# dropbox/divans

Hardware: AMD Instinct MI355X
Metric: MB/s encode+decode per GPU, 64 KiB metablocks; bit-exact vs CPU (higher is better)
Workload: dtype u16/u64 integer

## Files before the change

### divans_amd/csrc/capi.cpp

```cpp
#include <hip/hip_runtime.h>

#include <algorithm>
#include <atomic>
#include <cstdio>
#include <cstdlib>
#include <cstring>
#include <mutex>
#include <string>
#include <vector>

#include "../../include/divans_gpu.h"
#include "lit_kernels.h"
#include "lit_device.h"

using namespace divans_hip;

static thread_local std::string g_last_error;
static int fail(int code, const std::string& msg) { g_last_error = msg; return code; }
#define HIP_TRY(expr)                                                                              \
    do {                                                                                           \
        hipError_t e_ = (expr);                                                                    \
        if (e_ != hipSuccess)                                                                      \
            return fail(DIVANS_GPU_EHIP, std::string(#expr) + ": " + hipGetErrorString(e_));       \
    } while (0)
// ... 64 lines not shown
static void make_luts(uint8_t mode, uint8_t* lut0, uint8_t* lut1) {
    for (int i = 0; i < 256; ++i) {
        switch (mode) {
        case 3: lut0[i] = (uint8_t)(signed3(i) << 3); lut1[i] = signed3(i); break;
        case 2: lut0[i] = utf8_lut0(i); lut1[i] = utf8_lut1(i); break;
        case 1: lut0[i] = (uint8_t)(i >> 2); lut1[i] = 0; break;
        default: lut0[i] = (uint8_t)(i & 0x3f); lut1[i] = 0; break;
        }
    }
}

struct TableMem { int16_t* p = nullptr; size_t bytes = 0; std::vector<hipMemGenericAllocationHandle_t> chunks; size_t chunk_bytes = 0, va_bytes = 0; int device = 0; };

struct divans_gpu_codec {
    int device = 0;
    hipStream_t stream = nullptr;
    divans_lit_config cfg;
    LitGeometry geom;
    bool mix = false;
    uint32_t max_stream_len = 0;
    uint32_t num_cus = 256;
    uint32_t blocks = 0;
    uint32_t cache_high = 0, cache_low = 0;
    bool cache_unified = false;
    uint32_t decode_gen = 2;
#ifndef DIVANS_DM_AUTO_DEFAULT
#define DIVANS_DM_AUTO_DEFAULT 1
#endif
    bool dm_auto = DIVANS_DM_AUTO_DEFAULT != 0;
    uint32_t dm_log2 = 0, dm_shift = 0;
    uint32_t blocks2 = 0;
    uint32_t blocks_t = 0, t_log2 = 0, t_shift = 0;
    bool user_geometry = false;
    char last_decode_kernel[128] = "";
    uint32_t last_decode_grid = 0;
    uint8_t* d_stream_flags = nullptr;
    uint8_t* d_blob = nullptr;
    int16_t* d_tables = nullptr;  size_t tables_bytes = 0;
    TableMem tm;
    uint32_t byte_order = 0;
    uint8_t* d_rank = nullptr;
    bool rank_ready = false;
    uint32_t rans_split = 0;
    uint32_t table_candidates = 0; bool tables_tuned = false;
    bool eager_tune = false;
    divans_gpu_table_placement placement = {0u, 0u, 0.f, 0.f, 0.f, 0u, 0u};
    struct PlacementSearch {
        bool active = false, pending = false;
        uint32_t sig_streams = 0, sig_len = 0;
        TableMem best_tm;
        float best_ms = 0.f, worst_ms = 0.f;
        hipEvent_t e0 = nullptr, e1 = nullptr;
        uint64_t seq_at_measure = 0;
    } ps;
    uint64_t table_launch_seq = 0;
    uint32_t* d_sf = nullptr;     size_t sf_bytes = 0;
    uint32_t* d_status = nullptr;
    bool bucket_ok = false;
    bool bucket_mix_ok = false;
    uint32_t bucket_mix_batch = 32768;
    uint8_t* d_slots = nullptr; size_t slots_bytes = 0;
    uint64_t* d_slot_off = nullptr; size_t slot_off_cap = 0;
    std::vector<hipEvent_t> ev_span; size_t enc_spans = 0;
    float last_pack_ms = 0;
    uint32_t encode_path = 0;
    uint32_t last_encode_path = 0;
// ... 681 lines not shown
extern "C" int divans_gpu_codec_table_placement(divans_gpu_codec* c, divans_gpu_table_placement* out) {
    if (!c || !out) return fail(DIVANS_GPU_EINVAL, "null argument");
    *out = c->placement;
    out->policy_candidates = table_candidates_of(c);
    out->searching = (c->ps.active && !c->tables_tuned) ? 1u : 0u;
    return 0;
}

extern "C" int divans_gpu_table_memory(divans_gpu_table_memory_info* out) {
    if (!out) return fail(DIVANS_GPU_EINVAL, "null argument");
    out->va_reserved_bytes = g_va_reserved.load(); out->va_cap_bytes = g_va_cap.load();
    std::lock_guard<std::mutex> lock(g_table_pool_mu);
    out->idle_ranges = (uint32_t)g_table_pool.size(); out->idle_bytes = 0;
    for (const TableMem& m : g_table_pool) out->idle_bytes += m.va_bytes;
    return 0;
}
extern "C" void divans_gpu_set_table_va_cap(uint64_t bytes) { g_va_cap.store(bytes); }

static bool valid_cache_rows(uint32_t r) { return r == 0 || (r >= 16 && r <= 256 && (r & (r - 1)) == 0); }

extern "C" int divans_gpu_codec_set_geometry(divans_gpu_codec* c, uint32_t blocks, uint32_t cache_rows) {
    if (!c) return fail(DIVANS_GPU_EINVAL, "null codec");
    c->user_geometry = true;
    if (cache_rows != 0xffffffffu) {
        if (!valid_cache_rows(cache_rows)) return fail(DIVANS_GPU_EINVAL, "cache_rows must be 0 or a power of two in [16, 256]");
        if (cache_rows && c->geom.total_rows >= 0x7fffu) return fail(DIVANS_GPU_EINVAL, "row cache needs fewer than 32767 rows per stream");
        c->cache_high = cache_rows; c->cache_low = 0; c->cache_unified = cache_rows != 0;
#if DIVANS_WITH_EXPERIMENTAL_DECODERS
        c->decode_gen = 1;
#endif
    }
    if (blocks) {
        c->blocks = blocks;
        if (c->blocks2) {
            const uint32_t gen = c->decode_gen;
            int rc = set_decoder_impl(c, (c->dm_shift >> 31) ? 3 : 2, nullptr, nullptr, blocks, false); if (rc) return rc;
            c->decode_gen = gen;
        }
    }
    return 0;
}

extern "C" int divans_gpu_codec_set_split_cache(divans_gpu_codec* c, uint32_t high_rows, uint32_t low_rows) {
    if (!c) return fail(DIVANS_GPU_EINVAL, "null codec");
    if (!valid_cache_rows(high_rows) || !valid_cache_rows(low_rows)) return fail(DIVANS_GPU_EINVAL, "cache rows must be 0 or a power of two in [16, 256]");
    if (high_rows == 0 && low_rows != 0) return fail(DIVANS_GPU_EINVAL, "a low-nibble cache needs a high-nibble cache");
    if ((high_rows || low_rows) && c->geom.total_rows >= 0x7fffu) return fail(DIVANS_GPU_EINVAL, "row cache needs fewer than 32767 rows per stream");
    c->cache_high = high_rows; c->cache_low = low_rows; c->cache_unified = false;
#if DIVANS_WITH_EXPERIMENTAL_DECODERS
    c->decode_gen = 1;
#endif
    c->user_geometry = true;
    return 0;
}

extern "C" size_t divans_gpu_lit_encode_bound(size_t n) {
    const size_t nsym = 2 * n;
    const size_t nchunks = (nsym + 65535) / 65536;
    const size_t words = (15 * nsym + 31) / 32 + 2 * nchunks;
    const size_t bytes = 16 * nchunks + 4 * words;
    return (bytes + 15) & ~(size_t)15;
}

template <class Batch>
static void fill_bucket_batch(const divans_gpu_codec* c, uint32_t stream_len, const divans_lit_segment* d_segs, Batch& k) {
    k.stream_len = stream_len; k.max_stream_len = c->max_stream_len;
    k.pieces = bucket_pieces(c); k.slot = bucket_slot(c);
    k.segs = (const LitSegment*)d_segs; k.bt_first = c->geom.bt_first; k.n_btypes = c->geom.n_btypes; k.status = c->d_status;
}

template <class Batch, class Launch, class After>
static int bucket_sub_batches(divans_gpu_codec* c, Batch& k, uint32_t sub, const SfView& view, const uint8_t* d_in, const uint64_t* d_in_offsets,
                              const uint32_t* d_in_sizes, const uint32_t* d_seg_begin, uint32_t n_streams, Launch&& launch, After&& after) {
    HIP_TRY(hipEventRecord(c->ev[0], c->stream));
    for (uint32_t s0 = 0; s0 < n_streams; s0 += sub) {
        k.n_streams = std::min(sub, n_streams - s0);
        k.in = d_in_offsets ? d_in : d_in + (size_t)s0 * k.stream_len;
        k.in_offsets = d_in_offsets ? d_in_offsets + s0 : nullptr;
        k.in_sizes = d_in_sizes ? d_in_sizes + s0 : nullptr;
        k.seg_begin = d_seg_begin ? d_seg_begin + s0 : nullptr;
        if (int rc = launch(k)) return rc;
        if (int rc = after(s0, k.n_streams, view)) return rc;
    }
    return 0;
}

template <class After>
static int model_pass(divans_gpu_codec* c, const uint8_t* d_in, const uint64_t* d_in_offsets, const uint32_t* d_in_sizes,
                      uint32_t stream_len, uint32_t n_streams, const uint32_t* d_seg_begin, const divans_lit_segment* d_segs, After&& after) {
    int rc = maybe_learn_rank(c, d_in, d_in_offsets, d_in_sizes, n_streams, stream_len);
    if (rc) return rc;
    SfView view;
    const bool segs_ok = !d_segs || c->encode_path == 2u;
    if (use_bucket(c) && n_streams < (1u << 24) && segs_ok) {
        BucketBatch k;
        std::memset(&k, 0, sizeof(k));
        const uint32_t sub = std::min(n_streams, c->bucket_mix_batch);
        rc = ensure_bucket(c, sub, k); if (rc) return rc;
        fill_bucket_batch(c, stream_len, d_segs, k);
        k.sf = (uint32_t*)k.sfs; k.sf_stride = 2u * k.slot;
        k.inc = c->geom.inc0; k.lim = c->geom.lim0;
        c->last_encode_path = 2u;
        view.sf = k.sf; view.stride = k.sf_stride;
        view.spare = (uint8_t*)k.inv; view.spare_bytes = (size_t)sub * k.slot * 3u;
        return bucket_sub_batches(c, k, sub, view, d_in, d_in_offsets, d_in_sizes, d_seg_begin, n_streams,
                                  [&](const BucketBatch& kk) -> int { HIP_TRY(launch_bucket_model(kk, c->num_cus * 4u, c->stream)); return 0; }, after);
    }
    if (use_bucket_mix(c) && segs_ok) {
        MixBucketBatch k;
        std::memset(&k, 0, sizeof(k));
        uint32_t sub = std::min(n_streams, c->bucket_mix_batch);
        while ((rc = ensure_bucket_mix(c, sub, k)) == DIVANS_GPU_ENOMEM && sub > 1024u) { (void)hipGetLastError(); sub = (sub + 1u) / 2u; }
        if (rc) return rc;
        fill_bucket_batch(c, stream_len, d_segs, k);
        k.blob = c->d_blob; k.pos_stride = k.slot;
        k.sf = (uint32_t*)k.xs[0]; k.sf_stride = 2u * k.slot;
        k.inc0 = c->geom.inc0; k.lim0 = c->geom.lim0; k.inc2 = c->geom.inc2; k.lim2 = c->geom.lim2; k.inc3 = c->geom.inc3; k.lim3 = c->geom.lim3;
        c->last_encode_path = 3u;
        view.sf = k.sf; view.stride = k.sf_stride;
        view.spare = (uint8_t*)k.inv; view.spare_bytes = (size_t)sub * k.slot * 4u;
        return bucket_sub_batches(c, k, sub, view, d_in, d_in_offsets, d_in_sizes, d_seg_begin, n_streams,
                                  [&](const MixBucketBatch& kk) -> int { HIP_TRY(launch_bucket_mix_model(kk, c->num_cus, c->stream)); return 0; }, after);
    }
    rc = ensure_sf(c, n_streams); if (rc) return rc;
    rc = ensure_tables(c); if (rc) return rc;
    LitBatch b;
    std::memset(&b, 0, sizeof(b));
    b.blob = c->d_blob; b.geom = c->geom; b.tables = c->d_tables;
    b.n_streams = n_streams; b.stream_len = stream_len; b.max_stream_len = c->max_stream_len;
    b.in = d_in; b.in_offsets = d_in_offsets; b.in_sizes = d_in_sizes;
    b.sf = c->d_sf; b.status = c->d_status;
    b.seg_begin = d_seg_begin; b.segs = (const LitSegment*)d_segs;
    set_cache_fields(c, b);
    if (d_segs && b.cache_mode != 2u && b.cache_mode != 0u) return fail(DIVANS_GPU_EINVAL, "segment lists need the default (high-nibble-row) cache or none");
    HIP_TRY(hipEventRecord(c->ev[0], c->stream));
    ++c->table_launch_seq;
    c->last_encode_path = 1u;
    HIP_TRY(launch_model_encode(b, c->mix, c->blocks, c->stream));
    view.sf = c->d_sf; view.stride = 2u * c->max_stream_len;
    return after(0u, n_streams, view);
}

static int rans_event_pair(divans_gpu_codec* c, size_t i, hipEvent_t*& pair) {
    while (c->ev_rans.size() < 2u * (i + 1u)) {
        hipEvent_t e = nullptr;
        HIP_TRY(hipEventCreate(&e));
        c->ev_rans.push_back(e);
    }
    pair = &c->ev_rans[2u * i];
    return 0;
}

static int rans_pass(divans_gpu_codec* c, const SfView& v, uint32_t count, uint32_t stream_len, const uint32_t* d_in_sizes, uint8_t* out, uint64_t out_base,
                     uint64_t out_slot, uint64_t* d_out_offsets, uint32_t* d_out_sizes, uint32_t* d_chunk_bytes, uint32_t max_chunks, size_t& pairs) {
    const bool chunk_lanes = c->max_stream_len > 32768u && c->max_stream_len <= 65536u;
// ... 909 lines not shown
```

### divans_amd/csrc/lit_bucket.hip

```cpp
#include "lit_bucket_dev.h"

#ifndef DIVANS_BK_CHAIN_NO_STORES
#define DIVANS_BK_CHAIN_NO_STORES 0
#endif

namespace divans_hip {

template <bool SEG>
__global__ __launch_bounds__(BK_SORT_THREADS) void bucket_sort_kernel(const BucketBatch b) {
    __shared__ __attribute__((aligned(16))) unsigned long long staging64[BK_PIECE / 8u];
    uint8_t* staging = (uint8_t*)staging64;
    __shared__ __attribute__((aligned(16))) uint8_t piece_in[16 + BK_PIECE];
    __shared__ uint32_t hist[4][256];
    __shared__ uint32_t wsum[4];
    __shared__ uint8_t prev_of[SEG ? BK_PIECE : 1u];
    const uint32_t s = blockIdx.x / b.pieces, piece = blockIdx.x % b.pieces;
    const uint32_t tid = threadIdx.x, w = (uint32_t)__builtin_amdgcn_readfirstlane((int)(tid >> 6)), lane = tid & 63;
    const uint32_t len = b.in_sizes ? b.in_sizes[s] : b.stream_len;
    const uint8_t* in = b.in + (b.in_offsets ? b.in_offsets[s] : (uint64_t)s * b.stream_len);
    uint32_t* desc = b.desc + ((size_t)s * 256u + tid) * 8u + piece;
    const uint32_t base = piece * BK_PIECE;
    if (base >= len) {
        *desc = 0u;
        if (SEG && piece == 0u)
// ... 90 lines not shown
        uint32_t wbase = 0;
        if ((int)(threadIdx.x & 63u) == leader) wbase = atomicAdd(&cnt[c], (uint32_t)__popcll(m));
        wbase = (uint32_t)__builtin_amdgcn_readlane((int)wbase, leader);
        if (cls == c) local = wbase + lanes_below(m);
    }
    __syncthreads();
    if (threadIdx.x < BK_CLASSES) basev[threadIdx.x] = cnt[threadIdx.x] ? atomicAdd(&b.counters[threadIdx.x], cnt[threadIdx.x]) : 0u;
    __syncthreads();
    if (cls >= 0) b.tasks[(size_t)cls * cap + basev[cls] + local] = t;
}

constexpr uint32_t BK_LANE_DWORDS = 148;
constexpr uint32_t BK_DESC_DW = 136;
constexpr uint32_t BK_TAB_DW = 64 * BK_LANE_DWORDS;
__global__ __launch_bounds__(64) void bucket_chain_kernel(const BucketBatch b) {
    extern __shared__ __attribute__((aligned(16))) uint32_t lds32[];
    const uint32_t lane = threadIdx.x;
    uint32_t* my = lds32 + lane * BK_LANE_DWORDS;
    uint32_t* mydesc = my + BK_DESC_DW;
    uint32_t* tab = lds32 + BK_TAB_DW;
    const uint32_t inc = (uint32_t)b.inc; const int lim = b.lim;
    for (uint32_t i = lane; i < 128u; i += 64u) {
        tab[i] = bk_tab_entry(i, inc);
    }
    __syncthreads();
    const size_t pl = b.slot;
    const uint32_t cap = b.n_streams * 256u;
    BkTaskLists lists; lists.load(b.counters);
    const uint32_t total = lists.total();

    bool has_task = false, exhausted = false;
    uint32_t run_i = 0, nruns = 0, left = 0, idx = 0;
    u32x2* cur_sfs = b.sfs; const uint8_t* cur_sorted = b.sorted;
    uint32_t nt_stage = 0, nt_tid = 0;
    u32x4 nd0 = {0u, 0u, 0u, 0u}, nd1 = {0u, 0u, 0u, 0u};
    uint32_t win_cur = 0, win_end = 0, nxt_val = 0, nxt_w = 0;
    const uint32_t long_end = lists.ends[3];
    bool nxt_pending = false, drained = false;
    u32x2 e_next = {0u, 0u}; uint32_t m_next = 0;
    u32x2 pv0 = {0u, 0u}, pv1 = pv0, pv2 = pv0, pv3 = pv0, pv4 = pv0, pv5 = pv0, pv6 = pv0, pv7 = pv0;
    uint32_t m_prev = 0; u32x2* sfs_prev = b.sfs;

#define BK_OPAQUE(X) asm volatile("" : "+v"(X))
#define BK_BYTE(K, WORD, PV)                                                                            \
    if (((K - first) & 15u) < cnt) {                                                                    \
        const uint32_t byte_ = (WORD >> (8u * (K & 3u))) & 0xffu;                                       \
        const uint32_t hi = byte_ >> 4, lo = byte_ & 15u;                                               \
        uint32_t* rowl = my + 8u * (1u + hi);                                                           \
        BkRow H = bk_read(my, tab, hi), L = bk_read(rowl, tab, lo);                                     \
        const u32x2 v = {bk_pack(H, hi), bk_pack(L, lo)};                                               \
        bk_add(H); bk_add(L);                                                                           \
        bk_renorm_at(H, lim); bk_renorm_at(L, lim);                                                     \
        *(u32x4*)my = H.w0; *(u32x4*)(my + 4) = H.w1; *(u32x4*)rowl = L.w0; *(u32x4*)(rowl + 4) = L.w1; \
        PV = v;                                                                                         \
    }

    for (;;) {
        u32x2 e = e_next; const uint32_t m = m_next;
#if DIVANS_BK_CHAIN_NO_STORES
        asm volatile("" : : "v"(pv0), "v"(pv1), "v"(pv2), "v"(pv3), "v"(pv4), "v"(pv5), "v"(pv6), "v"(pv7), "v"(sfs_prev));
        if (false) {
#else
        if (m_prev & BK_VALID) {
#endif
            bk_store_group(sfs_prev, m_prev, pv0, pv1, pv2, pv3, pv4, pv5, pv6, pv7);
        }
        {
            const bool adv = has_task && left == 0u, more = run_i < nruns;
            const uint32_t d = mydesc[run_i & 7u];
            if (adv && more) { left = d >> 16; idx = d & 0xffffu; ++run_i; }
            if (adv && !more) has_task = false;
        }
        {
            const bool fetch_ = has_task && left != 0u;
            const uint32_t base = idx & ~7u, first_ = idx & 7u;
            const uint32_t cnt_ = left < 8u - first_ ? left : 8u - first_;
            const uint8_t* lp = fetch_ ? cur_sorted + base : b.sorted;
            e_next = *(const u32x2*)lp;
            m_next = fetch_ ? (base | (first_ << 16) | (cnt_ << 20) | BK_VALID) : 0u;
            idx += fetch_ ? cnt_ : 0u; left -= fetch_ ? cnt_ : 0u;
        }
        BK_OPAQUE(e);
        m_prev = m; sfs_prev = cur_sfs;
        if (m & BK_VALID) {
            const uint32_t first = (m >> 16) & 15u, cnt = (m >> 20) & 15u;
            BK_BYTE(0u, e.x, pv0) BK_BYTE(1u, e.x, pv1) BK_BYTE(2u, e.x, pv2) BK_BYTE(3u, e.x, pv3)
            BK_BYTE(4u, e.y, pv4) BK_BYTE(5u, e.y, pv5) BK_BYTE(6u, e.y, pv6) BK_BYTE(7u, e.y, pv7)
        }
        if (!has_task && !(m_next & BK_VALID) && nt_stage == 3u) {
            BK_OPAQUE(nd0); BK_OPAQUE(nd1);
            uint32_t n = 0;
            const uint32_t dsc[8] = {nd0.x, nd0.y, nd0.z, nd0.w, nd1.x, nd1.y, nd1.z, nd1.w};
#pragma unroll
            for (uint32_t j = 0; j < 8u; ++j) if (dsc[j] >> 16) { mydesc[n] = dsc[j] + j * BK_PIECE; ++n; }
            nruns = n; run_i = 0u;
            bk_rows_reset(my, 17u);
            cur_sfs = b.sfs + (size_t)(nt_tid >> 8) * pl; cur_sorted = b.sorted + (size_t)(nt_tid >> 8) * pl;
            left = 0u; has_task = true; nt_stage = 0u;
        }
        const bool want = nt_stage == 0u && !exhausted;
        if (nt_stage == 2u) nt_stage = 3u;
        else if (nt_stage == 1u) {
            BK_OPAQUE(nt_tid);
            const u32x4* dp = (const u32x4*)(b.desc + (size_t)nt_tid * 8u);
            nd0 = dp[0]; nd1 = dp[1];
            nt_stage = 2u;
        }
        const unsigned long long wm = __ballot(want);
        if (wm) {
            if (win_cur == win_end && nxt_pending) {
                BK_OPAQUE(nxt_val);
                const uint32_t basev = (uint32_t)__builtin_amdgcn_readfirstlane((int)nxt_val);
                nxt_pending = false;
                if (basev >= total) { drained = true; win_cur = win_end = total; }
                else { win_cur = basev; win_end = basev + nxt_w < total ? basev + nxt_w : total; }
            }
            const uint32_t avail = win_end - win_cur, asked = (uint32_t)__popcll(wm);
            const uint32_t rank = lanes_below(wm);
            if (want) {
                if (rank < avail) {
                    const uint32_t t = win_cur + rank;
                    nt_tid = *lists.at(b.tasks, cap, t);
                    nt_stage = 1u;
                } else if (drained) exhausted = true;
            }
            win_cur += asked < avail ? asked : avail;
        }
        const uint32_t want_w = win_end < long_end ? 64u : BK_WINDOW;
        if (!nxt_pending && !drained && win_end - win_cur < want_w / 2u) {
            nxt_w = want_w;
            if (lane == 0u) nxt_val = atomicAdd(&b.counters[BK_CLAIM], want_w);
            nxt_pending = true;
        }
        const bool done = !has_task && !(m_next & BK_VALID) && !(m_prev & BK_VALID) && nt_stage == 0u && exhausted;
        if (__ballot(!done) == 0ull) break;
    }
#undef BK_BYTE
#undef BK_OPAQUE
}

__global__ __launch_bounds__(1024) void bucket_unsort_kernel(const BucketBatch b) {
    __shared__ u32x2 buf[BK_PIECE];
    const uint32_t s = blockIdx.x / b.pieces, piece = blockIdx.x % b.pieces;
    const uint32_t len = b.in_sizes ? b.in_sizes[s] : b.stream_len;
    const uint32_t base = piece * BK_PIECE;
    if (base >= len) return;
    const uint32_t n = len - base < BK_PIECE ? len - base : BK_PIECE;
    const size_t pl = b.slot;
    const u32x2* src = b.sfs + (size_t)s * pl + base;
    for (uint32_t i = threadIdx.x; i < n; i += 1024u) buf[i] = __builtin_nontemporal_load(src + i);
    __syncthreads();
    const uint16_t* inv = b.inv + (size_t)s * pl + base;
    u32x2* dst = (u32x2*)(b.sf + (size_t)s * b.sf_stride) + base;
    for (uint32_t i = threadIdx.x; i < n; i += 1024u) dst[i] = buf[inv[i]];
}

__global__ __launch_bounds__(1024) void bucket_unsort32_kernel(const BucketBatch b) {
    __shared__ uint32_t buf[BK_PIECE];
    const uint32_t s = blockIdx.x / b.pieces, piece = blockIdx.x % b.pieces;
    const uint32_t len = b.in_sizes ? b.in_sizes[s] : b.stream_len;
    const uint32_t base = piece * BK_PIECE;
    if (base >= len) return;
    const uint32_t n = len - base < BK_PIECE ? len - base : BK_PIECE;
    const size_t pl = b.slot;
    const uint32_t* src = (const uint32_t*)b.sfs + (size_t)s * pl + base;
    const uint32_t n2 = (n + 1u) & ~1u;
    for (uint32_t i = 2u * threadIdx.x; i < n2; i += 2048u) *(u32x2*)(buf + i) = __builtin_nontemporal_load((const u32x2*)(src + i));
// ... 44 lines not shown
```

### divans_amd/csrc/lit_bucket_dev.h

```cpp
#ifndef DIVANS_LIT_BUCKET_DEV_H_
#define DIVANS_LIT_BUCKET_DEV_H_
#include "lit_device.h"

namespace divans_hip {

constexpr uint32_t BK_PIECE = 8192;
constexpr uint32_t BK_SORT_THREADS = 256;
constexpr uint32_t BK_VALID = 1u << 31;
constexpr uint32_t BK_WINDOW = 256;
constexpr uint32_t BK_CLASSES = 6;
constexpr uint32_t BK_CLAIM = 8;

__device__ __forceinline__ int bk_class_of(uint32_t tot) {
    return tot == 0u ? -1 : (tot >= 16384u ? 0 : (tot >= 8192u ? 1 : (tot >= 4096u ? 2 : (tot >= 2048u ? 3 : (tot >= 64u ? 4 : 5)))));
}
struct BkTaskLists {
    uint32_t ends[BK_CLASSES];
    __device__ __forceinline__ void load(const uint32_t* counters) {
        uint32_t acc = 0;
#pragma unroll
        for (uint32_t c = 0; c < BK_CLASSES; ++c) { acc += counters[c]; ends[c] = acc; }
    }
    __device__ __forceinline__ uint32_t total() const { return ends[BK_CLASSES - 1u]; }
    __device__ __forceinline__ const uint32_t* at(const uint32_t* tasks, uint32_t cap, uint32_t t) const {
// ... 119 lines not shown
template <class T>
__device__ __forceinline__ void bk_store_group(T* plane, uint32_t m, T r0, T r1, T r2, T r3, T r4, T r5, T r6, T r7) {
    T* dst = plane + (m & 0xffffu);
    const uint32_t pf = (m >> 16) & 15u, pc = (m >> 20) & 15u;
    if (pc == 8u) {
        bk_store_full(dst, r0, r1, r2, r3, r4, r5, r6, r7);
    } else {
        if (((0u - pf) & 15u) < pc) bk_store_one(dst + 0, r0);
        if (((1u - pf) & 15u) < pc) bk_store_one(dst + 1, r1);
        if (((2u - pf) & 15u) < pc) bk_store_one(dst + 2, r2);
        if (((3u - pf) & 15u) < pc) bk_store_one(dst + 3, r3);
        if (((4u - pf) & 15u) < pc) bk_store_one(dst + 4, r4);
        if (((5u - pf) & 15u) < pc) bk_store_one(dst + 5, r5);
        if (((6u - pf) & 15u) < pc) bk_store_one(dst + 6, r6);
        if (((7u - pf) & 15u) < pc) bk_store_one(dst + 7, r7);
    }
}

#define BK_OPAQUE(X) asm volatile("" : "+v"(X))

template <class K, class Batch>
__device__ __forceinline__ void bk_chain_loop(const typename K::Env env, const Batch b) {
    const uint32_t lane = threadIdx.x;
    uint32_t* my = env.my;
    uint32_t* mydesc = my + 8u * K::ROWS;
    const size_t pl = b.slot;
    const uint32_t cap = b.n_streams * 256u;
    BkTaskLists lists; lists.load(b.counters);
    const uint32_t total = lists.total();

    bool has_task = false, exhausted = false;
    uint32_t run_i = 0, nruns = 0, left = 0, idx = 0;
    typename K::Slot cur = K::slot(b, 0u); const auto* cur_sorted = b.sorted;
    uint32_t nt_stage = 0, nt_tid = 0;
    u32x4 nd0 = {0u, 0u, 0u, 0u}, nd1 = {0u, 0u, 0u, 0u};
    uint32_t win_cur = 0, win_end = 0, nxt_val = 0, nxt_w = 0;
    const uint32_t long_end = lists.ends[3];
    bool nxt_pending = false, drained = false;
    typename K::Group e_next = {}; uint32_t m_next = 0;
    typename K::Out out = {};
    uint32_t m_prev = 0; typename K::Slot prev = cur;

    for (;;) {
        typename K::Group e = e_next; const uint32_t m = m_next;
        if (m_prev & BK_VALID) K::store(prev, m_prev, out);
        {
            const bool adv = has_task && left == 0u, more = run_i < nruns;
            const uint32_t d = mydesc[run_i & 7u];
            if (adv && more) { left = d >> 16; idx = d & 0xffffu; ++run_i; }
            if (adv && !more) has_task = false;
        }
        {
            const bool fetch_ = has_task && left != 0u;
            const uint32_t base = idx & ~7u, first_ = idx & 7u;
            const uint32_t cnt_ = left < 8u - first_ ? left : 8u - first_;
            const auto* lp = fetch_ ? cur_sorted + base : b.sorted;
            e_next = *(const typename K::Group*)lp;
            m_next = fetch_ ? (base | (first_ << 16) | (cnt_ << 20) | BK_VALID) : 0u;
            idx += fetch_ ? cnt_ : 0u; left -= fetch_ ? cnt_ : 0u;
        }
        BK_OPAQUE(e);
        m_prev = m; prev = cur;
        if (m & BK_VALID) out = K::code(env, e, (m >> 16) & 15u, (m >> 20) & 15u, out);
        if (!has_task && !(m_next & BK_VALID) && nt_stage == 3u) {
            BK_OPAQUE(nd0); BK_OPAQUE(nd1);
            uint32_t n = 0;
            const uint32_t dsc[8] = {nd0.x, nd0.y, nd0.z, nd0.w, nd1.x, nd1.y, nd1.z, nd1.w};
#pragma unroll
            for (uint32_t j = 0; j < 8u; ++j) if (dsc[j] >> 16) { mydesc[n] = dsc[j] + j * BK_PIECE; ++n; }
            nruns = n; run_i = 0u;
            bk_rows_reset(my, K::ROWS);
            const size_t off = (size_t)(nt_tid >> 8) * pl;
            cur = K::slot(b, off); cur_sorted = b.sorted + off;
            left = 0u; has_task = true; nt_stage = 0u;
        }
        const bool want = nt_stage == 0u && !exhausted;
        if (nt_stage == 2u) nt_stage = 3u;
        else if (nt_stage == 1u) {
            BK_OPAQUE(nt_tid);
            const u32x4* dp = (const u32x4*)(b.desc + (size_t)nt_tid * 8u);
            nd0 = dp[0]; nd1 = dp[1];
            nt_stage = 2u;
        }
        const unsigned long long wm = __ballot(want);
        if (wm) {
            if (win_cur == win_end && nxt_pending) {
                BK_OPAQUE(nxt_val);
                const uint32_t basev = (uint32_t)__builtin_amdgcn_readfirstlane((int)nxt_val);
                nxt_pending = false;
                if (basev >= total) { drained = true; win_cur = win_end = total; }
                else { win_cur = basev; win_end = basev + nxt_w < total ? basev + nxt_w : total; }
            }
            const uint32_t avail = win_end - win_cur, asked = (uint32_t)__popcll(wm);
            const uint32_t rank = lanes_below(wm);
            if (want) {
                if (rank < avail) {
                    const uint32_t t = win_cur + rank;
                    nt_tid = *lists.at(b.tasks, cap, t);
                    nt_stage = 1u;
                } else if (drained) exhausted = true;
            }
            win_cur += asked < avail ? asked : avail;
        }
        const uint32_t want_w = win_end < long_end ? 64u : BK_WINDOW;
        if (!nxt_pending && !drained && win_end - win_cur < want_w / 2u) {
            nxt_w = want_w;
            if (lane == 0u) nxt_val = atomicAdd(&b.counters[BK_CLAIM], want_w);
            nxt_pending = true;
        }
        const bool done = !has_task && !(m_next & BK_VALID) && !(m_prev & BK_VALID) && nt_stage == 0u && exhausted;
        if (__ballot(!done) == 0ull) break;
    }
}
#undef BK_OPAQUE

}
#endif
```

### divans_amd/csrc/lit_bucket_mix.hip

```cpp
#include "lit_bucket_dev.h"

namespace divans_hip {

constexpr uint32_t MX_CHAIN_WAVES = 3;

template <int MODEL> struct MxGeom {
    static constexpr uint32_t NH = MODEL == 0 ? 8u : 1u;
    static constexpr uint32_t NR = NH + 16u;
    static constexpr uint32_t LANE_DW = MODEL == 0 ? 204u : 148u;
    static constexpr uint32_t LDS_BYTES = (64u * LANE_DW + 256u) * 4u;
};

template <int MODEL, bool SEG>
__global__ __launch_bounds__(BK_SORT_THREADS) void mix_sort_kernel(const MixBucketBatch b) {
    __shared__ __attribute__((aligned(16))) uint16_t staging[BK_PIECE];
    __shared__ __attribute__((aligned(16))) uint8_t piece_in[16 + BK_PIECE];
    __shared__ uint16_t kp[BK_PIECE];
    __shared__ uint32_t hist[4][256];
    __shared__ uint32_t scan[256];
    __shared__ uint8_t lut1c[256], ctxf[2048], slot_of[2048];
    const uint32_t s = blockIdx.x / b.pieces, piece = blockIdx.x % b.pieces;
    const uint32_t tid = threadIdx.x, w = tid >> 6, lane = tid & 63;
    const uint32_t len = b.in_sizes ? b.in_sizes[s] : b.stream_len;
    const uint8_t* in = b.in + (b.in_offsets ? b.in_offsets[s] : (uint64_t)s * b.stream_len);
// ... 302 lines not shown
                const uint32_t sf = bk_pack(R, s);
                rec[0] = (int)(sf & 0xffffu); rec[1] = (int)(sf >> 16); rec[2] = (int)s;
            } else if (kind == 6u) {
                bk_rows_reset(rows[0], 2u);
                for (int i = 0; i < 16; ++i) rec[i] = r0[i];
            } else if (kind == 8u && op.y < 2u) {
                ((uint16_t*)rows[op.y])[op.z & 15u] = (uint16_t)op.w;
                for (int i = 0; i < 16; ++i) rec[i] = ((const uint16_t*)rows[op.y])[i];
            } else if (kind == 10u) {
                const BkRow C = bk_read(rows[0], tab, sym), S = bk_read(rows[1], tab, sym);
                const uint32_t cm_x = (uint32_t)C.chi | (sym ? (uint32_t)C.cprev << 16 : 0u), st_x = (uint32_t)S.chi | (sym ? (uint32_t)S.cprev << 16 : 0u);
                uint32_t mf = 0u;
                const uint32_t sf = mix_nibble<true>(w, st_x, S.w1.w >> 16, cm_x, C.w1.w >> 16, &mf);
                rec[0] = (int)(sf & 0xffffu); rec[1] = (int)(sf >> 16); rec[2] = (int)sym; rec[3] = (int)(mf & 0xffffu); rec[4] = (int)(mf >> 16);
                rec[5] = w.w0; rec[6] = w.w1; rec[7] = w.norm;
            }
            if (kind == 5u || (kind == 8u && op.y >= 2u)) { rec[0] = w.w0; rec[1] = w.w1; rec[2] = w.norm; }
#pragma unroll
            for (int i = 0; i < 16; ++i) out[(size_t)k * 16u + (uint32_t)i] = rec[i];
        }
        if (kind == 10u) {
            w.w0 = __builtin_amdgcn_readfirstlane(w.w0); w.w1 = __builtin_amdgcn_readfirstlane(w.w1); w.norm = __builtin_amdgcn_readfirstlane(w.norm);
        }
    }
}

hipError_t launch_selftest_cdf_ops_bucket(const uint32_t* d_ops, uint32_t n, int32_t* d_out, hipStream_t st) {
    hipLaunchKernelGGL(cdf_ops_selftest_bucket_kernel, dim3(1), dim3(64), 0, st, (const u32x4*)d_ops, n, d_out);
    return hipGetLastError();
}

static void launch_mix_sort_seg(int model, const MixBucketBatch& b, hipStream_t st);

hipError_t launch_bucket_mix_model(const MixBucketBatch& b, uint32_t num_cus, hipStream_t st) {
    BucketBatch v;
    v.in = b.in; v.in_offsets = b.in_offsets; v.in_sizes = b.in_sizes;
    v.n_streams = b.n_streams; v.stream_len = b.stream_len; v.max_stream_len = b.max_stream_len; v.pieces = b.pieces;
    v.slot = b.slot; v.sf_stride = 2u * b.pos_stride;
    v.sorted = nullptr; v.inv = b.inv; v.desc = b.desc; v.sfs = nullptr; v.sf = nullptr; v.tasks = b.tasks; v.counters = b.counters;
    v.inc = 0; v.lim = 0;
    v.seg_begin = nullptr; v.segs = nullptr; v.bt_first = 0; v.n_btypes = 0; v.status = nullptr;
    for (int model = 0; model < 2; ++model) {
        hipError_t e = hipMemsetAsync(b.counters, 0, 64, st);
        if (e != hipSuccess) return e;
        if (b.pieces < 8u) {
            e = hipMemsetAsync(b.desc, 0, (size_t)b.n_streams * 256u * 8u * sizeof(uint32_t), st);
            if (e != hipSuccess) return e;
        }
        if (model == 0) {
            if (b.segs) launch_mix_sort_seg(0, b, st);
            else hipLaunchKernelGGL((mix_sort_kernel<0, false>), dim3(b.n_streams * b.pieces), dim3(BK_SORT_THREADS), 0, st, b);
            launch_bucket_tasks(v, st);
            hipLaunchKernelGGL(mix_chain_kernel<0>, dim3(num_cus * MX_CHAIN_WAVES), dim3(64), MxGeom<0>::LDS_BYTES, st, b);
        } else {
            if (b.segs) launch_mix_sort_seg(1, b, st);
            else hipLaunchKernelGGL((mix_sort_kernel<1, false>), dim3(b.n_streams * b.pieces), dim3(BK_SORT_THREADS), 0, st, b);
            launch_bucket_tasks(v, st);
            hipLaunchKernelGGL(mix_chain_kernel<1>, dim3(num_cus * MX_CHAIN_WAVES), dim3(64), MxGeom<1>::LDS_BYTES, st, b);
        }
        v.sfs = b.xs[model]; v.sf = (uint32_t*)b.xs[model]; v.sf_stride = 2u * b.pos_stride;
        launch_bucket_unsort(v, st);
        v.sfs = (bk_u32x2*)b.maxes[model]; v.sf = b.maxes[model]; v.sf_stride = b.pos_stride;
        launch_bucket_unsort32(v, st);
    }
    if ((b.n_streams + 31u) / 32u > num_cus * 4u) hipLaunchKernelGGL(mix_weights_kernel<2>, dim3((b.n_streams + 31u) / 32u), dim3(64), 0, st, b);
    else hipLaunchKernelGGL(mix_weights_kernel<1>, dim3((b.n_streams + 31u) / 32u), dim3(64), 0, st, b);
    return hipGetLastError();
}

static void launch_mix_sort_seg(int model, const MixBucketBatch& b, hipStream_t st) {
    if (model == 0) hipLaunchKernelGGL((mix_sort_kernel<0, true>), dim3(b.n_streams * b.pieces), dim3(BK_SORT_THREADS), 0, st, b);
    else hipLaunchKernelGGL((mix_sort_kernel<1, true>), dim3(b.n_streams * b.pieces), dim3(BK_SORT_THREADS), 0, st, b);
}

}
```

### divans_amd/csrc/lit_kernels.h

```cpp
#ifndef DIVANS_LIT_KERNELS_H_
#define DIVANS_LIT_KERNELS_H_
#include <hip/hip_runtime.h>
#include <stdint.h>

namespace divans_hip {

constexpr int LIT_THREADS = 256;
constexpr int RANS_THREADS = 64;

constexpr uint32_t LIT_BLOB_LUT1CLASS = 0;
constexpr uint32_t LIT_BLOB_CTXF = 256;
constexpr uint32_t LIT_CTXF_BYTES = 2048;
constexpr uint32_t LIT_MAX_BTYPES = 8;
constexpr uint32_t LIT_BLOB_MAX_BYTES = 256 + LIT_CTXF_BYTES * LIT_MAX_BTYPES + 8192;

struct LitGeometry {
    uint32_t nctx;
    uint32_t low_width;
    uint32_t plane0, plane1, plane2;
    uint32_t low_base;
    uint32_t cm_base;
    uint32_t total_rows;
    int32_t mm_uniform;
    int32_t ctx_const;
// ... 60 lines not shown
    int32_t inc, lim;
    const uint32_t* seg_begin;
    const LitSegment* segs;
    uint32_t bt_first, n_btypes;
    uint32_t* status;
};
hipError_t launch_bucket_model(const BucketBatch& b, uint32_t chain_blocks, hipStream_t st);
void launch_bucket_tasks(const BucketBatch& b, hipStream_t st);
void launch_bucket_unsort(const BucketBatch& b, hipStream_t st);
void launch_bucket_unsort32(const BucketBatch& b, hipStream_t st);

struct MixBucketBatch {
    const uint8_t* in; const uint64_t* in_offsets; const uint32_t* in_sizes;
    uint32_t n_streams, stream_len, max_stream_len;
    uint32_t pieces;
    uint32_t slot;
    uint32_t pos_stride;
    uint32_t sf_stride;
    const uint8_t* blob;
    uint16_t* sorted;
    uint16_t* inv;
    uint32_t* desc;
    uint32_t* tasks;
    uint32_t* counters;
    bk_u32x2* xs[2];
    uint32_t* maxes[2];
    uint32_t* sf;
    int32_t inc0, lim0, inc2, lim2, inc3, lim3;
    const uint32_t* seg_begin;
    const LitSegment* segs;
    uint32_t bt_first, n_btypes;
    uint32_t* status;
};
hipError_t launch_bucket_mix_model(const MixBucketBatch& b, uint32_t num_cus, hipStream_t st);

uint32_t lit_lds_bytes(const LitBatch& b);
hipError_t launch_model_encode(const LitBatch& b, bool mix, uint32_t blocks, hipStream_t st);
hipError_t launch_rans_encode(const RansBatch& b, hipStream_t st);
hipError_t launch_decode(const LitBatch& b, bool mix, uint32_t blocks, hipStream_t st);
hipError_t launch_decode2(const LitBatch& b, bool mix, uint32_t blocks, hipStream_t st);
void lit_decode_kernel_name(const LitBatch& b, bool mix, char* buf, size_t cap);
void lit_decode2_kernel_name(const LitBatch& b, bool mix, char* buf, size_t cap);
uint32_t lit_decode2_effective_caches(uint32_t dm_log2, bool mix, bool seg);
uint32_t lit_decode2_stream_lds(uint32_t dm_log2);
#ifndef DIVANS_WITH_EXPERIMENTAL_DECODERS
#define DIVANS_WITH_EXPERIMENTAL_DECODERS 0
#endif
#if DIVANS_WITH_EXPERIMENTAL_DECODERS
hipError_t launch_decode_t(const LitBatch& b, bool mix, uint32_t blocks, hipStream_t st);
hipError_t launch_selftest_cdf_ops_t(const uint32_t* d_ops, uint32_t n, int32_t* d_out, hipStream_t st);
void lit_decode_t_kernel_name(const LitBatch& b, bool mix, char* buf, size_t cap);
uint32_t lit_decode_t_stream_lds(uint32_t dm_log2, bool mix);
#endif
hipError_t launch_pack(const uint8_t* slots, const uint64_t* src_off, const uint32_t* sizes, uint32_t n, uint8_t* packed,
                       uint64_t* dst_off, uint64_t* total, hipStream_t st, bool accumulate = false, uint64_t cap = ~0ull, uint32_t* status = nullptr);
hipError_t launch_learn_byte_rank(const uint8_t* data, const uint64_t* offsets, const uint32_t* sizes, uint32_t n_streams, uint32_t stream_len,
                                  uint32_t sample_streams, uint32_t sample_len, uint8_t* rank, hipStream_t st);
hipError_t launch_row_replay(const LitBatch& b, bool mix, uint32_t blocks, hipStream_t st);
hipError_t launch_selftest_division(unsigned long long* d_mismatches, hipStream_t st);
hipError_t launch_selftest_cdf_ops(const uint32_t* d_ops, uint32_t n, int32_t* d_out, hipStream_t st);
hipError_t launch_selftest_cdf_ops2(const uint32_t* d_ops, uint32_t n, int32_t* d_out, hipStream_t st);
hipError_t launch_selftest_cdf_ops_bucket(const uint32_t* d_ops, uint32_t n, int32_t* d_out, hipStream_t st);

}
#endif
```

Measured before the change: 14880.

## Add one-deep task descriptor queue to bucket chain kernels; cap chain grid

Restructures the per-wave task fetch state machine in the bucket and mix-bucket chain loops. A descriptor that has finished loading is now moved into a one-entry queue, so the next task claim and its descriptor load can start while the current task is still running, instead of waiting in a stage-3 hold. The aim is to hide task-fetch latency between tasks, at the cost of more registers per lane. Separately, a user-set block count now also caps the chain kernel grid size.

```diff
diff --git a/divans_amd/csrc/capi.cpp b/divans_amd/csrc/capi.cpp
--- a/divans_amd/csrc/capi.cpp
+++ b/divans_amd/csrc/capi.cpp
@@ -120,6 +120,7 @@
     uint32_t blocks2 = 0;
     uint32_t blocks_t = 0, t_log2 = 0, t_shift = 0;
     bool user_geometry = false;
+    uint32_t chain_grid_cap = 0;
     char last_decode_kernel[128] = "";
     uint32_t last_decode_grid = 0;
     uint8_t* d_stream_flags = nullptr;
@@ -867,6 +868,7 @@
     }
     if (blocks) {
         c->blocks = blocks;
+        c->chain_grid_cap = blocks;
         if (c->blocks2) {
             const uint32_t gen = c->decode_gen;
             int rc = set_decoder_impl(c, (c->dm_shift >> 31) ? 3 : 2, nullptr, nullptr, blocks, false); if (rc) return rc;
@@ -896,6 +898,8 @@
     const size_t bytes = 16 * nchunks + 4 * words;
     return (bytes + 15) & ~(size_t)15;
 }
+
+static uint32_t chain_grid(const divans_gpu_codec* c, uint32_t own) { return c->chain_grid_cap ? std::min(own, c->chain_grid_cap) : own; }
 
 template <class Batch>
 static void fill_bucket_batch(const divans_gpu_codec* c, uint32_t stream_len, const divans_lit_segment* d_segs, Batch& k) {
@@ -939,7 +943,7 @@
         view.sf = k.sf; view.stride = k.sf_stride;
         view.spare = (uint8_t*)k.inv; view.spare_bytes = (size_t)sub * k.slot * 3u;
         return bucket_sub_batches(c, k, sub, view, d_in, d_in_offsets, d_in_sizes, d_seg_begin, n_streams,
-                                  [&](const BucketBatch& kk) -> int { HIP_TRY(launch_bucket_model(kk, c->num_cus * 4u, c->stream)); return 0; }, after);
+                                  [&](const BucketBatch& kk) -> int { HIP_TRY(launch_bucket_model(kk, chain_grid(c, c->num_cus * 4u), c->stream)); return 0; }, after);
     }
     if (use_bucket_mix(c) && segs_ok) {
         MixBucketBatch k;
@@ -955,7 +959,7 @@
         view.sf = k.sf; view.stride = k.sf_stride;
         view.spare = (uint8_t*)k.inv; view.spare_bytes = (size_t)sub * k.slot * 4u;
         return bucket_sub_batches(c, k, sub, view, d_in, d_in_offsets, d_in_sizes, d_seg_begin, n_streams,
-                                  [&](const MixBucketBatch& kk) -> int { HIP_TRY(launch_bucket_mix_model(kk, c->num_cus, c->stream)); return 0; }, after);
+                                  [&](const MixBucketBatch& kk) -> int { HIP_TRY(launch_bucket_mix_model(kk, c->num_cus, c->chain_grid_cap, c->stream)); return 0; }, after);
     }
     rc = ensure_sf(c, n_streams); if (rc) return rc;
     rc = ensure_tables(c); if (rc) return rc;
diff --git a/divans_amd/csrc/lit_bucket.hip b/divans_amd/csrc/lit_bucket.hip
--- a/divans_amd/csrc/lit_bucket.hip
+++ b/divans_amd/csrc/lit_bucket.hip
@@ -146,8 +146,9 @@
     bool has_task = false, exhausted = false;
     uint32_t run_i = 0, nruns = 0, left = 0, idx = 0;
     u32x2* cur_sfs = b.sfs; const uint8_t* cur_sorted = b.sorted;
-    uint32_t nt_stage = 0, nt_tid = 0;
-    u32x4 nd0 = {0u, 0u, 0u, 0u}, nd1 = {0u, 0u, 0u, 0u};
+    uint32_t nt_stage = 0, nt_tid = 0, q_tid = 0;
+    u32x4 nd0 = {0u, 0u, 0u, 0u}, nd1 = nd0, qd0 = nd0, qd1 = nd0;
+    bool q_full = false;
     uint32_t win_cur = 0, win_end = 0, nxt_val = 0, nxt_w = 0;
     const uint32_t long_end = lists.ends[3];
     bool nxt_pending = false, drained = false;
@@ -179,6 +180,47 @@
 #endif
             bk_store_group(sfs_prev, m_prev, pv0, pv1, pv2, pv3, pv4, pv5, pv6, pv7);
         }
+        if (nt_stage == 2u && !q_full) {
+            qd0 = nd0; qd1 = nd1; q_tid = nt_tid;
+            q_full = true; nt_stage = 0u;
+        }
+        {
+            const bool want = nt_stage == 0u && !exhausted && !q_full;
+            if (nt_stage == 1u) {
+                BK_OPAQUE(nt_tid);
+                const u32x4* dp = (const u32x4*)(b.desc + (size_t)nt_tid * 8u);
+                nd0 = dp[0]; nd1 = dp[1];
+                nt_stage = 2u;
+            }
+            const unsigned long long wm = __ballot(want);
+            if (wm) {
+                if (win_cur == win_end && nxt_pending) {
+                    BK_OPAQUE(nxt_val);
+                    const uint32_t basev = (uint32_t)__builtin_amdgcn_readfirstlane((int)nxt_val);
+                    nxt_pending = false;
+                    if (basev >= total) { drained = true; win_cur = win_end = total; }
+                    else { win_cur = basev; win_end = basev + nxt_w < total ? basev + nxt_w : total; }
+                }
+                const uint32_t avail = win_end - win_cur, asked = (uint32_t)__popcll(wm);
+                const uint32_t rank = lanes_below(wm);
+                if (want) {
+                    if (rank < avail) {
+                        const uint32_t t = win_cur + rank;
+                        nt_tid = *lists.at(b.tasks, cap, t);
+                        nt_stage = 1u;
+                    } else if (drained) exhausted = true;
+                }
+                win_cur += asked < avail ? asked : avail;
+            }
+            const uint32_t want_w = win_end < long_end ? 64u : BK_WINDOW;
+            if (!nxt_pending && !drained && win_end - win_cur < want_w / 2u) {
+                nxt_w = want_w;
+                uint32_t claim = BK_CLAIM;
+                BK_OPAQUE(claim);
+                if (lane == 0u) nxt_val = atomicAdd(b.counters + claim, want_w);
+                nxt_pending = true;
+            }
+        }
         {
             const bool adv = has_task && left == 0u, more = run_i < nruns;
             const uint32_t d = mydesc[run_i & 7u];
@@ -201,52 +243,18 @@
             BK_BYTE(0u, e.x, pv0) BK_BYTE(1u, e.x, pv1) BK_BYTE(2u, e.x, pv2) BK_BYTE(3u, e.x, pv3)
             BK_BYTE(4u, e.y, pv4) BK_BYTE(5u, e.y, pv5) BK_BYTE(6u, e.y, pv6) BK_BYTE(7u, e.y, pv7)
         }
-        if (!has_task && !(m_next & BK_VALID) && nt_stage == 3u) {
-            BK_OPAQUE(nd0); BK_OPAQUE(nd1);
+        if (!has_task && !(m_next & BK_VALID) && q_full) {
+            BK_OPAQUE(qd0); BK_OPAQUE(qd1);
             uint32_t n = 0;
-            const uint32_t dsc[8] = {nd0.x, nd0.y, nd0.z, nd0.w, nd1.x, nd1.y, nd1.z, nd1.w};
+            const uint32_t dsc[8] = {qd0.x, qd0.y, qd0.z, qd0.w, qd1.x, qd1.y, qd1.z, qd1.w};
 #pragma unroll
             for (uint32_t j = 0; j < 8u; ++j) if (dsc[j] >> 16) { mydesc[n] = dsc[j] + j * BK_PIECE; ++n; }
             nruns = n; run_i = 0u;
             bk_rows_reset(my, 17u);
-            cur_sfs = b.sfs + (size_t)(nt_tid >> 8) * pl; cur_sorted = b.sorted + (size_t)(nt_tid >> 8) * pl;
-            left = 0u; has_task = true; nt_stage = 0u;
-        }
-        const bool want = nt_stage == 0u && !exhausted;
-        if (nt_stage == 2u) nt_stage = 3u;
-        else if (nt_stage == 1u) {
-            BK_OPAQUE(nt_tid);
-            const u32x4* dp = (const u32x4*)(b.desc + (size_t)nt_tid * 8u);
-            nd0 = dp[0]; nd1 = dp[1];
-            nt_stage = 2u;
-        }
-        const unsigned long long wm = __ballot(want);
-        if (wm) {
-            if (win_cur == win_end && nxt_pending) {
-                BK_OPAQUE(nxt_val);
-                const uint32_t basev = (uint32_t)__builtin_amdgcn_readfirstlane((int)nxt_val);
-                nxt_pending = false;
-                if (basev >= total) { drained = true; win_cur = win_end = total; }
-                else { win_cur = basev; win_end = basev + nxt_w < total ? basev + nxt_w : total; }
-            }
-            const uint32_t avail = win_end - win_cur, asked = (uint32_t)__popcll(wm);
-            const uint32_t rank = lanes_below(wm);
-            if (want) {
-                if (rank < avail) {
-                    const uint32_t t = win_cur + rank;
-                    nt_tid = *lists.at(b.tasks, cap, t);
-                    nt_stage = 1u;
-                } else if (drained) exhausted = true;
-            }
-            win_cur += asked < avail ? asked : avail;
-        }
-        const uint32_t want_w = win_end < long_end ? 64u : BK_WINDOW;
-        if (!nxt_pending && !drained && win_end - win_cur < want_w / 2u) {
-            nxt_w = want_w;
-            if (lane == 0u) nxt_val = atomicAdd(&b.counters[BK_CLAIM], want_w);
-            nxt_pending = true;
-        }
-        const bool done = !has_task && !(m_next & BK_VALID) && !(m_prev & BK_VALID) && nt_stage == 0u && exhausted;
+            cur_sfs = b.sfs + (size_t)(q_tid >> 8) * pl; cur_sorted = b.sorted + (size_t)(q_tid >> 8) * pl;
+            left = 0u; has_task = true; q_full = false;
+        }
+        const bool done = !has_task && !(m_next & BK_VALID) && !(m_prev & BK_VALID) && nt_stage == 0u && !q_full && exhausted;
         if (__ballot(!done) == 0ull) break;
     }
 #undef BK_BYTE
diff --git a/divans_amd/csrc/lit_bucket_dev.h b/divans_amd/csrc/lit_bucket_dev.h
--- a/divans_amd/csrc/lit_bucket_dev.h
+++ b/divans_amd/csrc/lit_bucket_dev.h
@@ -175,8 +175,9 @@
     bool has_task = false, exhausted = false;
     uint32_t run_i = 0, nruns = 0, left = 0, idx = 0;
     typename K::Slot cur = K::slot(b, 0u); const auto* cur_sorted = b.sorted;
-    uint32_t nt_stage = 0, nt_tid = 0;
-    u32x4 nd0 = {0u, 0u, 0u, 0u}, nd1 = {0u, 0u, 0u, 0u};
+    uint32_t nt_stage = 0, nt_tid = 0, q_tid = 0;
+    u32x4 nd0 = {0u, 0u, 0u, 0u}, nd1 = nd0, qd0 = nd0, qd1 = nd0;
+    bool q_full = false;
     uint32_t win_cur = 0, win_end = 0, nxt_val = 0, nxt_w = 0;
     const uint32_t long_end = lists.ends[3];
     bool nxt_pending = false, drained = false;
@@ -187,6 +188,47 @@
     for (;;) {
         typename K::Group e = e_next; const uint32_t m = m_next;
         if (m_prev & BK_VALID) K::store(prev, m_prev, out);
+        if (nt_stage == 2u && !q_full) {
+            qd0 = nd0; qd1 = nd1; q_tid = nt_tid;
+            q_full = true; nt_stage = 0u;
+        }
+        {
+            const bool want = nt_stage == 0u && !exhausted && !q_full;
+            if (nt_stage == 1u) {
+                BK_OPAQUE(nt_tid);
+                const u32x4* dp = (const u32x4*)(b.desc + (size_t)nt_tid * 8u);
+                nd0 = dp[0]; nd1 = dp[1];
+                nt_stage = 2u;
+            }
+            const unsigned long long wm = __ballot(want);
+            if (wm) {
+                if (win_cur == win_end && nxt_pending) {
+                    BK_OPAQUE(nxt_val);
+                    const uint32_t basev = (uint32_t)__builtin_amdgcn_readfirstlane((int)nxt_val);
+                    nxt_pending = false;
+                    if (basev >= total) { drained = true; win_cur = win_end = total; }
+                    else { win_cur = basev; win_end = basev + nxt_w < total ? basev + nxt_w : total; }
+                }
+                const uint32_t avail = win_end - win_cur, asked = (uint32_t)__popcll(wm);
+                const uint32_t rank = lanes_below(wm);
+                if (want) {
+                    if (rank < avail) {
+                        const uint32_t t = win_cur + rank;
+                        nt_tid = *lists.at(b.tasks, cap, t);
+                        nt_stage = 1u;
+                    } else if (drained) exhausted = true;
+                }
+                win_cur += asked < avail ? asked : avail;
+            }
+            const uint32_t want_w = win_end < long_end ? 64u : BK_WINDOW;
+            if (!nxt_pending && !drained && win_end - win_cur < want_w / 2u) {
+                nxt_w = want_w;
+                uint32_t claim = BK_CLAIM;
+                BK_OPAQUE(claim);
+                if (lane == 0u) nxt_val = atomicAdd(b.counters + claim, want_w);
+                nxt_pending = true;
+            }
+        }
         {
             const bool adv = has_task && left == 0u, more = run_i < nruns;
             const uint32_t d = mydesc[run_i & 7u];
@@ -205,53 +247,19 @@
         BK_OPAQUE(e);
         m_prev = m; prev = cur;
         if (m & BK_VALID) out = K::code(env, e, (m >> 16) & 15u, (m >> 20) & 15u, out);
-        if (!has_task && !(m_next & BK_VALID) && nt_stage == 3u) {
-            BK_OPAQUE(nd0); BK_OPAQUE(nd1);
+        if (!has_task && !(m_next & BK_VALID) && q_full) {
+            BK_OPAQUE(qd0); BK_OPAQUE(qd1);
             uint32_t n = 0;
-            const uint32_t dsc[8] = {nd0.x, nd0.y, nd0.z, nd0.w, nd1.x, nd1.y, nd1.z, nd1.w};
+            const uint32_t dsc[8] = {qd0.x, qd0.y, qd0.z, qd0.w, qd1.x, qd1.y, qd1.z, qd1.w};
 #pragma unroll
             for (uint32_t j = 0; j < 8u; ++j) if (dsc[j] >> 16) { mydesc[n] = dsc[j] + j * BK_PIECE; ++n; }
             nruns = n; run_i = 0u;
             bk_rows_reset(my, K::ROWS);
-            const size_t off = (size_t)(nt_tid >> 8) * pl;
+            const size_t off = (size_t)(q_tid >> 8) * pl;
             cur = K::slot(b, off); cur_sorted = b.sorted + off;
-            left = 0u; has_task = true; nt_stage = 0u;
-        }
-        const bool want = nt_stage == 0u && !exhausted;
-        if (nt_stage == 2u) nt_stage = 3u;
-        else if (nt_stage == 1u) {
-            BK_OPAQUE(nt_tid);
-            const u32x4* dp = (const u32x4*)(b.desc + (size_t)nt_tid * 8u);
-            nd0 = dp[0]; nd1 = dp[1];
-            nt_stage = 2u;
-        }
-        const unsigned long long wm = __ballot(want);
-        if (wm) {
-            if (win_cur == win_end && nxt_pending) {
-                BK_OPAQUE(nxt_val);
-                const uint32_t basev = (uint32_t)__builtin_amdgcn_readfirstlane((int)nxt_val);
-                nxt_pending = false;
-                if (basev >= total) { drained = true; win_cur = win_end = total; }
-                else { win_cur = basev; win_end = basev + nxt_w < total ? basev + nxt_w : total; }
-            }
-            const uint32_t avail = win_end - win_cur, asked = (uint32_t)__popcll(wm);
-            const uint32_t rank = lanes_below(wm);
-            if (want) {
-                if (rank < avail) {
-                    const uint32_t t = win_cur + rank;
-                    nt_tid = *lists.at(b.tasks, cap, t);
-                    nt_stage = 1u;
-                } else if (drained) exhausted = true;
-            }
-            win_cur += asked < avail ? asked : avail;
-        }
-        const uint32_t want_w = win_end < long_end ? 64u : BK_WINDOW;
-        if (!nxt_pending && !drained && win_end - win_cur < want_w / 2u) {
-            nxt_w = want_w;
-            if (lane == 0u) nxt_val = atomicAdd(&b.counters[BK_CLAIM], want_w);
-            nxt_pending = true;
-        }
-        const bool done = !has_task && !(m_next & BK_VALID) && !(m_prev & BK_VALID) && nt_stage == 0u && exhausted;
+            left = 0u; has_task = true; q_full = false;
+        }
+        const bool done = !has_task && !(m_next & BK_VALID) && !(m_prev & BK_VALID) && nt_stage == 0u && !q_full && exhausted;
         if (__ballot(!done) == 0ull) break;
     }
 }
diff --git a/divans_amd/csrc/lit_bucket_mix.hip b/divans_amd/csrc/lit_bucket_mix.hip
--- a/divans_amd/csrc/lit_bucket_mix.hip
+++ b/divans_amd/csrc/lit_bucket_mix.hip
@@ -358,7 +358,8 @@
 
 static void launch_mix_sort_seg(int model, const MixBucketBatch& b, hipStream_t st);
 
-hipError_t launch_bucket_mix_model(const MixBucketBatch& b, uint32_t num_cus, hipStream_t st) {
+hipError_t launch_bucket_mix_model(const MixBucketBatch& b, uint32_t num_cus, uint32_t chain_grid_cap, hipStream_t st) {
+    const uint32_t own = num_cus * MX_CHAIN_WAVES, chain_grid = chain_grid_cap && chain_grid_cap < own ? chain_grid_cap : own;
     BucketBatch v;
     v.in = b.in; v.in_offsets = b.in_offsets; v.in_sizes = b.in_sizes;
     v.n_streams = b.n_streams; v.stream_len = b.stream_len; v.max_stream_len = b.max_stream_len; v.pieces = b.pieces;
@@ -377,12 +378,12 @@
             if (b.segs) launch_mix_sort_seg(0, b, st);
             else hipLaunchKernelGGL((mix_sort_kernel<0, false>), dim3(b.n_streams * b.pieces), dim3(BK_SORT_THREADS), 0, st, b);
             launch_bucket_tasks(v, st);
-            hipLaunchKernelGGL(mix_chain_kernel<0>, dim3(num_cus * MX_CHAIN_WAVES), dim3(64), MxGeom<0>::LDS_BYTES, st, b);
+            hipLaunchKernelGGL(mix_chain_kernel<0>, dim3(chain_grid), dim3(64), MxGeom<0>::LDS_BYTES, st, b);
         } else {
             if (b.segs) launch_mix_sort_seg(1, b, st);
             else hipLaunchKernelGGL((mix_sort_kernel<1, false>), dim3(b.n_streams * b.pieces), dim3(BK_SORT_THREADS), 0, st, b);
             launch_bucket_tasks(v, st);
-            hipLaunchKernelGGL(mix_chain_kernel<1>, dim3(num_cus * MX_CHAIN_WAVES), dim3(64), MxGeom<1>::LDS_BYTES, st, b);
+            hipLaunchKernelGGL(mix_chain_kernel<1>, dim3(chain_grid), dim3(64), MxGeom<1>::LDS_BYTES, st, b);
         }
         v.sfs = b.xs[model]; v.sf = (uint32_t*)b.xs[model]; v.sf_stride = 2u * b.pos_stride;
         launch_bucket_unsort(v, st);
diff --git a/divans_amd/csrc/lit_kernels.h b/divans_amd/csrc/lit_kernels.h
--- a/divans_amd/csrc/lit_kernels.h
+++ b/divans_amd/csrc/lit_kernels.h
@@ -116,7 +116,7 @@
     uint32_t bt_first, n_btypes;
     uint32_t* status;
 };
-hipError_t launch_bucket_mix_model(const MixBucketBatch& b, uint32_t num_cus, hipStream_t st);
+hipError_t launch_bucket_mix_model(const MixBucketBatch& b, uint32_t num_cus, uint32_t chain_grid_cap, hipStream_t st);
 
 uint32_t lit_lds_bytes(const LitBatch& b);
 hipError_t launch_model_encode(const LitBatch& b, bool mix, uint32_t blocks, hipStream_t st);
```

New measurement: 14960 (median of 6 runs). Within noise of the previous version (+0.5%).
